# AnnSeidel/genometools

Hardware: AMD Instinct MI355X
Metric: Gbp/s ESA build (suf+lcp+bwt), 3 Gbp DNA, 1/2/4/8 MI355X; bit-exact vs CPU (higher is better)
Workload: dtype u64; 1 GPU; human-like DNA (2% N, 24 seqs, repeats) n=3000000000 seed=43 -suf -lcp -bwt (BASELINE.json configs[2]); parallelism=1 device, pair_suffixes=341032298, tied_suffixes=390540711, refine_rounds=9, maxbranchdepth=8256

## Files before the change

genometools_amd/csrc/esa_engine.hip:

```cpp
#include <stdarg.h>
#include <stdlib.h>
#include <chrono>
#include <type_traits>
#include <utility>
#include <vector>
#include "../../include/gtamd_esa.h"
#include "esa_prims.h"
#include "esa_devutil.h"
#include "esa_own.h"

static thread_local char g_err[1024] = "";
void gtamd_set_error(const char *fmt, ...) {
  va_list ap;
  va_start(ap, fmt);
  vsnprintf(g_err, sizeof g_err, fmt, ap);
  va_end(ap);
}
extern "C" const char *gtamd_esa_last_error(void) { return g_err; }

extern "C" int gtamd_device_count(void) {
  GTAMD_ABI_BEGIN
  int n = 0;
  if (hipGetDeviceCount(&n) != hipSuccess) return 0;
  return n;
// ... 2412 lines not shown
  bool msd_pack = true;
  u32 msd_pack_cap = MD_CAP;
  u32 msd_bin_limit = MD_BIN_LIMIT_DEFAULT;
  bool fused_pass0 = true;
  bool force_wide = false;
  bool no_pairs = false;
  bool no_small_groups = false;
  int apply_early = 2;
  u64 apply_wgs = 0;
  bool apply_wgs_given = false;
  int rank_window_bits = RW_BITS;
  bool rank_all_windows = false;
  bool win_filter_global = false;
  int pair_chunk = 0;
  u32 round_stride = 1536;
  bool debug = false;
};

static Switches read_switches() {
  Switches sw;
  auto flag = [](const char *name, char c) {
    const char *e = getenv(name);
    return e != nullptr && e[0] == c;
  };
  if (const char *e = getenv("GTAMD_MSD")) sw.msd = e[0] == '1';
  sw.msd_part_off = flag("GTAMD_MSD", '0');
  if (const char *e = getenv("GTAMD_MSD_CBITS")) {
    const int v = atoi(e);
    if (v >= 0 && v <= 8) sw.msd_cbits = v;
  }
// ... 23 lines not shown
    sw.apply_wgs_given = true;
  }
  if (const char *e = getenv("GTAMD_RANK_WINDOW_BITS")) {
    const int v = atoi(e);
    if (v >= 2 && v <= RW_BITS) sw.rank_window_bits = v;
  }
  sw.rank_all_windows = flag("GTAMD_RANK_ALL_WINDOWS", '1');
  sw.win_filter_global = flag("GTAMD_WIN_FILTER_LDS", '0');
  if (const char *e = getenv("GTAMD_PAIR_CHUNK")) {
    const int v = atoi(e);
    if (v >= 4 && v <= 1024) sw.pair_chunk = v;
  }
  if (const char *e = getenv("GTAMD_ROUND_STRIDE")) {
    const int v = atoi(e);
    if (v >= RT_STRIDE_MIN && v <= RT_TILE) sw.round_stride = (u32) v;
  }
  sw.debug = getenv("GTAMD_DEBUG") != nullptr;
  return sw;
}

struct gtamd_esa_ctx {
  int device = 0;
  u32 sigma = 0;
  int bits = 0;
  u64 max_n = 0, n = 0, N = 0;
  int readmode = 0;
  Stream st, st2;
  Event ev_sorted, ev_emitted, ev_applied;
  DevBuf tb_own, sp_own;
  Text text = {};
// ... 789 lines not shown
template <int BITS, bool WIDE>
struct Build {
  using K = Key<BITS>;
  using P = typename std::conditional<WIDE, u64, u32>::type;
  static constexpr u64 RANKREC = 1 + sizeof(P) / 4;
  static constexpr u64 ISA_CHUNK = 1ull << 27;

  gtamd_esa_ctx *const c;
  const Switches &sw;
  u32 want;
  const bool dist;
  const u64 N, n;
  const u32 R;
  const hipStream_t st;
  const bool debug;

  u32 prefixlength = 0;
  bool long_prefix = false, want_suf = false, want_lcp = false, want_bwt = false;
  bool msd = false;
  bool msd_part = false;
  bool fused_pass0 = false;

  int fail = 0;

  u64 NL, index_offset = 0;
  Tiles tl;
  u64 Tn;
  u64 prev_key = 0;
  int has_prev = 0;

// ... 141 lines not shown
    u32 *lhead = nullptr;
    u64 list_cap = 0;
  } rk;

  struct RankTable {
    u32 *rank32, *heads, *ppos, *phead, *qhead, *qpos;
    const u32 *spos;
    bool heads_array;
    int wmax, pb, wb, split;
    int fb;
    GroupHeadValues headgen;
  } rt;

  Build(gtamd_esa_ctx *ctx, const Switches &switches, u32 want_, bool dist_)
      : c(ctx), sw(switches), want(want_), dist(dist_), N(ctx->N), n(ctx->n), R(ctx->numparts),
        st(ctx->st), debug(switches.debug), NL(ctx->N), Tn(ctx->N) {
    tl.T = N;
    tl.self = c->part;
  }

  int run() {
    TRY(plan());
    if (!dist) TRY(first_sort_whole());
    else if (msd_part) TRY(first_sort_filtered());
    else TRY(first_sort_exchanged());
    TRY(finish_first_sort());
    TRY(count_ties());
    if (anyties > 0) {
      TRY(count_tied_words());
      bool settled = false;
      TRY(settle_few_ties(&settled));
// ... 33 lines not shown
    TRY(fork_second_stream());
    if (NL > 0) {
      k_finalize<BITS, P><<<stride_grid(div_up(NL, FIN_TILE)), FIN_THREADS, 0, c->st2>>>(
          skey, sa, NL, prefixlength, d_suf, d_lcp, d_bwt, nullptr,
          c->d_stats, prev_key, has_prev, index_offset);
      HIP_TRY(hipGetLastError());
    }
    HIP_TRY(hipEventRecord(c->ev_emitted, c->st2));
    return 0;
  }

  int tie_words(const u64 *bits) {
    if (NL > 0) {
      k_tie_words<<<(u32) nwb, 256, 0, st>>>(bits, nwords, wd.cntw, wd.headw);
      HIP_TRY(hipGetLastError());
      TRY(scan_u32(SCAN_SUM, wd.cntw, wd.offw, nwb, false, wd.scanws, st));
      TRY(scan_u32(SCAN_MAX, wd.headw, wd.carry, nwords, false, wd.scanws, st));
    }
    k_total<<<1, 1, 0, st>>>(wd.offw, wd.cntw, NL > 0 ? nwb : 0, c->d_stats);
    HIP_TRY(hipGetLastError());
    TRY(fetch_stats(c));
    return 0;
  }

  u64 direct_limit() const { return NL / 512 > 4096 ? NL / 512 : 4096; }
  int direct_ties(const u32 *uidx0, const u32 *ugrp, bool clear_fallback) {
    TRY(launch_emission());
    HIP_TRY(hipStreamWaitEvent(st, c->ev_emitted, 0));
    if (clear_fallback) HIP_TRY(hipMemsetAsync(&c->d_stats->dfallback, 0, 4, st));
    if (m0 > 0) {
      k_direct_ties<BITS, P><<<(u32) div_up(m0, 256), 256, 0, st>>>(
          c->text, uidx0, ugrp, m0, sa, d_suf, d_lcp, d_bwt, want_lcp,
// ... 24 lines not shown
    if (R > 1 && (c->comm_allgather == nullptr || c->comm_alltoallv == nullptr)) {
      gtamd_set_error("a part build needs the collective callbacks "
                      "(gtamd_esa_set_comm)");
      return -1;
    }
    memset(&c->timing, 0, sizeof c->timing);
    memset(&c->stats, 0, sizeof c->stats);
    c->alloc_ms = 0;
    c->llv_pairs = 0;
    if (!dist && !WIDE && !(want & GTAMD_WANT_BCK) && N >= 64 && (BITS == 2 || (prefixlength <= 9 && c->sigma <= 20))) {
      msd = sw.msd >= 0 ? sw.msd == 1 : N >= (1ull << 25);
    }
    if (dist && BITS == 2) msd_part = !sw.msd_part_off;
    fused_pass0 = !dist && !msd && BITS == 2 && sw.fused_pass0;
    if (debug)
      fprintf(stderr, "gtamd: part %u: run: parts=%u positions=%d first_sort=%s pass0=%s\n", c->part, R,
              WIDE ? 64 : 32, msd || msd_part ? "msd" : "lsd",
              dist || msd || BITS != 2 ? "none" : (fused_pass0 ? "fused" : "plain"));
    return 0;
  }

  int first_sort_whole() {
    TRY(ensure_workspace(c, N, want, false));
    HIP_TRY(hipMemsetAsync(c->d_stats, 0, sizeof(Stats), st));
    HIP_TRY(hipEventRecord(c->ev[EV_START], st));
    if (msd) {
      TRY(msd_sort_emit<BITS == 5 ? 1 : 0>(c, sw, want, prefixlength, N, N, nullptr, &msd_sa, &msd_fkey, &msd_fval,
                                           &msd_local));
      HIP_TRY(hipEventRecord(c->ev_emitted, st));
    } else if (fused_pass0) {
      const u32 ntiles = (u32) div_up(N, KP_TILE);
      k_dc_hist_dna<<<ntiles, KP_THREADS, 0, st>>>(c->text, N, c->rws.as<u32>());
      HIP_TRY(hipGetLastError());
// ... 51 lines not shown
    if (NL >= SINGLE_LIMIT) {
      set_slice_error(NL);
      return -1;
    }
    const u64 cap = NL > Tn ? NL : Tn;
    TRY(ensure_workspace(c, cap, want, true));
    if (WIDE) TRY(ensure_buf(c, c->posw, (NL + 8) * 8, "the positions of the part's suffixes"));
    msd_sa = c->v0.as<u32>();
    msd_fkey = c->k1.as<u64>();
    msd_fval = c->v1.as<u32>();
    if (NL == 0) {
      HIP_TRY(hipMemsetAsync(c->tiebits.p, 0, 16, st));
      HIP_TRY(hipEventRecord(c->ev[EV_KEYS], st));
      return 0;
    }
    TRY(scan_u32(SCAN_SUM, tkeep, tkeep, ntT, false, tscan, st));
    u64 *ck = c->isa_tmp.as<u64>();
    HIP_TRY(hipMemsetAsync(acc + 3, 0, 8, st));
    if (WIDE)
      k_part_filter<u64><<<ntT, MS_THREADS, 0, st>>>(c->text, N, lo, hi, binbelow, tkeep, ck,
                                                    c->posw.as<u64>(), acc + 3);
    else
      k_part_filter<u32><<<ntT, MS_THREADS, 0, st>>>(c->text, N, lo, hi, binbelow, tkeep, ck,
                                                    c->v1.as<u32>(), acc + 3);
    HIP_TRY(hipGetLastError());
    MsdPartSrc src;
    src.ck = ck;
    src.cp32 = WIDE ? nullptr : c->v1.as<u32>();
    src.index_offset = index_offset;
    src.prev_key = acc + 3;
    src.has_prev = has_prev;
// ... 111 lines not shown
              (unsigned long long) index_offset, WIDE ? " (64-bit positions)" : "");
    if (dist && !msd_part) TRY(comm_allgather(c, fail, nullptr, nullptr, 0));
    if (!msd) HIP_TRY(hipEventRecord(c->ev[EV_KEYS], st));

    static_assert((64 - Key<2>::LOW_BITS) % 8 == 0, "whole passes over the DNA prefix");
    int shifts[16], widths[16];
    const int np = passes_for(pass0_done ? K::LOW_BITS : K::DSHIFT, 64, shifts, widths);
    u64 *ka = pass0_done ? c->k1.as<u64>() : c->k0.as<u64>(),
        *kb = pass0_done ? c->k0.as<u64>() : c->k1.as<u64>();
    u32 *va = pass0_done ? c->v1.as<u32>() : c->v0.as<u32>(),
        *vb = pass0_done ? c->v0.as<u32>() : c->v1.as<u32>();
    if (!msd) {
      hipEvent_t evs[2 * 16];
      for (int i = 0; i < 2 * 16; i++) evs[i] = c->ev_scatter[i];
      TRY(radix_sort_pairs<u64, u32>(ka, va, kb, vb, NL, shifts, widths, np,
                                c->rws.as<u32>(), st, evs, &nev));
    }
    skey = (np & 1) ? kb : ka;
    u32 *sa32 = (np & 1) ? vb : va;
    fkey = (np & 1) ? ka : kb;
    fval = (np & 1) ? va : vb;
    if (msd) {
      skey = nullptr;
      sa32 = msd_sa;
      fkey = msd_fkey;
      fval = msd_fval;
    }
    HIP_TRY(hipEventRecord(c->ev[EV_SORTED], st));

    if (want & GTAMD_WANT_BCK) TRY(build_bcktab<BITS>(c, skey, sa32, NL, prefixlength, st));

// ... 82 lines not shown
    return 0;
  }

  int pair_path() {
    TRY(ensure_buf(c, c->tiebits2, (nwords + 2) * 8, "the tie bitmap"));
    tiebits2 = c->tiebits2.as<u64>();
    const bool no_pairs = sw.no_pairs;
    const bool no_small = no_pairs || sw.no_small_groups;
    u64 nsrec = 0;
    if (NL > 0) {
      if (no_pairs) {
        HIP_TRY(hipMemcpyAsync(tiebits2, tiebits, nwords * 8, hipMemcpyDeviceToDevice, st));
      } else {
        k_pair_words<<<(u32) nwb, 256, 0, st>>>(tiebits, nwords, wd.pcnt, wd.scnt, wd.rcnt, tiebits2);
        HIP_TRY(hipGetLastError());
        TRY(scan_u32(SCAN_SUM, wd.pcnt, wd.poff, nwb, false, wd.scanws, st));
        TRY(scan_u32(SCAN_SUM, wd.scnt, wd.soff, nwb, false, wd.scanws, st));
        TRY(scan_u32(SCAN_SUM, wd.rcnt, wd.roff, nwb, false, wd.scanws, st));
        k_total2<<<1, 1, 0, st>>>(wd.poff, wd.pcnt, nwb, c->d_stats);
        k_total3<<<1, 1, 0, st>>>(wd.soff, wd.scnt, nwb, c->d_stats);
        k_total<<<1, 1, 0, st>>>(wd.roff, wd.rcnt, nwb, c->d_stats);
        HIP_TRY(hipGetLastError());
        TRY(fetch_stats(c));
        npairs = c->h_stats->count2;
        nsmall = c->h_stats->count3;
        nsrec = c->h_stats->count;
      }
    }
    if (no_small || nsrec > NL / 8 || npairs + nsrec >= SINGLE_LIMIT) { nsmall = 0; nsrec = 0; }
    nrec = npairs + nsrec;
    apply_early = sw.apply_early;
    {
      Bump sz = {nullptr, 0};
// ... 10 lines not shown
    nbl = bits_for(NL ? NL - 1 : 0);
    pn = passes_for(0, nb, ps, pw);
    pair_swp = npairs > 0 ? pl.swp : nullptr;
    if (nrec == 0) return 0;
    if (npairs > 0) {
      k_pair_emit<P><<<(u32) div_up(nwords, 256), 256, 0, st>>>(tiebits, nwords, wd.poff, sa, pl.pk_a,
                                                               pl.pv_a, pl.pidx);
      HIP_TRY(hipGetLastError());
    }
    if (nsmall > 0) {
      k_small_emit<P><<<(u32) div_up(nwords, 256), 256, 0, st>>>(
          tiebits, nwords, wd.soff, wd.roff, sa, npairs, pl.sidx, pl.ssize, pl.srec, pl.pk_a, pl.pv_a);
      HIP_TRY(hipGetLastError());
    }
    TRY(radix_sort_pairs<P, u64>(pl.pk_a, pl.pv_a, pl.pk_b, pl.pv_b, nrec, ps, pw, pn, pl.prws, st,
                                 nullptr, nullptr));
    const P *pk_sorted = (pn & 1) ? pl.pk_b : pl.pk_a;
    const u64 *pv_sorted = (pn & 1) ? pl.pv_b : pl.pv_a;
    TRY(launch_emission());
    int pair_chunk = (int) (nrec >> 20 < 16 ? 16 : (nrec >> 20 > 128 ? 128 : nrec >> 20));
    if (sw.pair_chunk > 0) pair_chunk = sw.pair_chunk;
    pair_chunk = (pair_chunk + PR_LINE - 1) / PR_LINE * PR_LINE;
    if (debug)
      fprintf(stderr, "gtamd: part %u: pair resolve: records=%llu chunk=%d grid=%u\n", c->part,
              (unsigned long long) nrec, pair_chunk,
              stride_grid(div_up(div_up(nrec, (u64) pair_chunk), 256)));
    k_pair_resolve<BITS, P><<<stride_grid(div_up(div_up(nrec, (u64) pair_chunk), 256)), 256, 0, st>>>(
        c->text, pk_sorted, pv_sorted, nrec, npairs, sa, pl.pres, c->d_stats, pair_chunk);
    HIP_TRY(hipGetLastError());
    if (npairs > 0) {
      k_pair_swapbits<<<(u32) nwb, 256, 0, st>>>(tiebits, nwords, wd.poff, pl.pres, pl.swp);
// ... 160 lines not shown
  int rank_windows(const u32 *in_pos, const u32 *in_head, u32 *a_pos, u32 *a_head, u32 *b_pos,
                   u32 *b_head, u64 count, int bits, int pb, int split, u64 span, const u32 *list,
                   int fb, u32 nsel, u64 M) {
    const u32 *wpos = in_pos, *whead = in_head;
    if (pb > 0) {
      const int s0 = bits - pb, w0 = pb > 8 ? pb - 8 : pb;
      if (in_head != nullptr)
        TRY(radix_partition_u32(in_pos, in_head, a_pos, a_head, count, s0, w0, wd.pws, st));
      else
        TRY(radix_pass_group_heads(in_pos, rt.headgen, a_pos, a_head, count, s0, w0, wd.pws, st));
      wpos = a_pos; whead = a_head;
    }
    if (pb > 8) {
      const int s1 = bits - 8, w1 = 8;
      TRY(radix_sort_pairs<u32, u32>(a_pos, a_head, b_pos, b_head, count, &s1, &w1, 1, wd.pws, st,
                                     nullptr, nullptr));
      wpos = b_pos; whead = b_head;
    }
    const int wb = bits - pb;
    const u32 nbuckets = (u32) div_up(count, 1ull << wb);
    const u32 grid = split == 2 ? ((nbuckets + 7u) / 8u) * 16u : nbuckets;
    k_rank_window<<<grid, RW_THREADS, 0, st>>>(wpos, whead, span, wb, split, nbuckets, rt.rank32,
                                               list, fb, nsel, M);
    HIP_TRY(hipGetLastError());
    return 0;
  }

  int build_rank(bool first) {
    u64 nsel = 0;
    if (rk.windows) {
      k_win_select<<<1, 1024, 0, st>>>(rk.w_need, rk.w_built, rk.nww, rk.w_sel, rk.w_list, rk.w_pref, c->d_stats);
// ... 331 lines not shown
      if (c->h_stats->count2 != 0) TRY(build_rank(false));
    }
    const u32 rt_stride = sw.round_stride;
    const u32 g = (u32) div_up(m, 256);
    const u32 ntiles = (u32) div_up(m, rt_stride);
    const u32 nfb = (u32) div_up(m, RT_TILE);
    u32 *tilecnt = ar.koff, *tileoff = ar.koff + nfb + 16;
    HIP_TRY(hipMemsetAsync(ar.flagbits, 0, (u64) nfb * (RT_TILE / 8), st));
    k_tile_starts<<<ntiles / 256 + 1, 256, 0, st>>>(ar.ugrp, m, ntiles, rt_stride, ar.tstart);
    HIP_TRY(hipGetLastError());
    k_round_tile<P><<<ntiles, RT_THREADS, 0, st>>>(
        ar.uidx, ar.upos, ar.ugrp, ar.k2, m, ar.cvo, ar.hv, ar.tstart, ar.flagbits, dist ? nullptr : rank, h, n);
    HIP_TRY(hipGetLastError());
    k_flag_count<<<nfb / 256 + 1, 256, 0, st>>>(ar.flagbits, m, nfb, tilecnt);
    HIP_TRY(hipGetLastError());
    TRY(scan_u32(SCAN_SUM, tilecnt, tileoff, nfb, false, ar.scanws2, st));
    k_total<<<1, 1, 0, st>>>(tileoff, tilecnt, nfb, c->d_stats);
    HIP_TRY(hipGetLastError());
    TRY(fetch_stats(c));
    const u64 nf = c->h_stats->count;
    if (debug)
      fprintf(stderr, "gtamd: part %u round %u: %llu entries in groups across tile borders "
              "(%u tiles, stride %u)\n", c->part, rounds, (unsigned long long) nf, ntiles, rt_stride);
    if (nf > 0) {
      k_flag_gather<P><<<nfb, RT_THREADS, 0, st>>>(ar.flagbits, tileoff, ar.ugrp, ar.k2, ar.upos, m, ar.fk2,
                                                     ar.fk2s_a, ar.fgrp, ar.fpos, ar.fj, ar.perm_a);
      HIP_TRY(hipGetLastError());
      TRY(radix_sort_pairs<P, u32>(ar.fk2s_a, ar.perm_a, ar.fk2s_b, ar.perm_b, nf, ps, pw, pn, ar.rws2, st,
                                   nullptr, nullptr));
      u32 *perm1 = (pn & 1) ? ar.perm_b : ar.perm_a, *permx = (pn & 1) ? ar.perm_a : ar.perm_b;
      const u32 gf = (u32) div_up(nf, 256);
      k_gather_u32<<<gf, 256, 0, st>>>(ar.fgrp, perm1, nf, ar.gk_a);
      HIP_TRY(hipGetLastError());
      TRY(radix_sort_pairs<u32, u32>(ar.gk_a, perm1, ar.gk_b, permx, nf, s.gs, s.gw, s.gn, ar.rws2, st,
                                     nullptr, nullptr));
      const u32 *perm2 = (s.gn & 1) ? permx : perm1;
      k_flag_heads<P><<<gf, 256, 0, st>>>(perm2, ar.fgrp, ar.fk2, ar.fpos, ar.uidx, ar.fj, nf, ar.fhv, ar.cvs);
      HIP_TRY(hipGetLastError());
      TRY(scan_u32(SCAN_MAX, ar.fhv, ar.fhv, nf, true, ar.scanws2, st));
      k_flag_scatter<P><<<gf, 256, 0, st>>>(ar.cvs, ar.fhv, ar.fj, nf, ar.cvo, ar.hv);
      HIP_TRY(hipGetLastError());
    }
    u32 *bcnt = ar.koff, *boffs = ar.koff + g + 16;
    k_round_apply<P><<<g, 256, 0, st>>>(ar.cvo, ar.hv, ar.uidx, ar.ugrp, m, index_offset, sa,
                                        dist ? nullptr : rank, ar.keep, bcnt);
    HIP_TRY(hipGetLastError());
    TRY(scan_u32(SCAN_SUM, bcnt, boffs, g, false, ar.scanws2, st));
    k_round_compact<P><<<g, 256, 0, st>>>(ar.keep, boffs, bcnt, ar.uidx, ar.cvo, ar.hv, m, ar.uidx2,
                                          ar.upos2, ar.ugrp2, c->d_stats);
    HIP_TRY(hipGetLastError());
    TRY(fetch_stats(c));
    s.m = c->h_stats->count;
    s.h *= 2;
    if (dist) {
      s.ru.cval = ar.cvo; s.ru.gnew = ar.hv; s.ru.ugrp = ar.ugrp; s.ru.index_offset = index_offset;
      s.ru.tl = tl; s.ru.isa = isa; s.ru.soff = ar.xoff; s.ru.srank = ar.xrank;
      s.m_upd = m;
      TRY(dest_count(c, s.ru, s.m_upd, ar.xdest_u, ar.xbc_u, ar.xbo_u, ar.scanws2, 1));
      s.rq.upos = ar.upos2; s.rq.h = s.h;
      TRY(dest_count(c, s.rq, s.m, ar.xdest_q, ar.xbc_q, ar.xbo_q, ar.scanws2, 0));
    }
    std::swap(ar.uidx, ar.uidx2);
// ... 12 lines not shown
      else lcpfull = c->isa_tmp.as<u32>();
    }
    if (!apply_early) TRY(launch_apply(st));
    const u32 g0 = (u32) div_up(m0, 256);
    u32 *bcnt0 = ar.koff, *boff0 = ar.koff + g0 + 16;
    if (m0 > 0) {
      TRY(fork_second_stream());
      k_fix_basic<BITS, P><<<g0, 256, 0, c->st2>>>(c->text, ar.uidx0, m0, sa, d_suf, d_bwt,
                                                   c->d_stats, index_offset);
      HIP_TRY(hipGetLastError());
      HIP_TRY(hipEventRecord(c->ev_emitted, c->st2));
    }
    if (want_lcp && m0 > 0) {
      k_tied_counts<<<g0, 256, 0, st>>>(ar.uidx0, m0, tiebits2, bcnt0);
      HIP_TRY(hipGetLastError());
      TRY(scan_u32(SCAN_SUM, bcnt0, boff0, g0, false, ar.scanws2, st));
      k_total<<<1, 1, 0, st>>>(boff0, bcnt0, g0, c->d_stats);
      HIP_TRY(hipGetLastError());
      TRY(fetch_stats(c));
      const u64 m1 = c->h_stats->count;
      k_lcp_pairs<P><<<g0, 256, 0, st>>>(boff0, tiebits2, ar.uidx0, sa, m0, ar.lk_a, ar.lv_a);
      HIP_TRY(hipGetLastError());
      TRY(radix_sort_pairs<P, u32>(ar.lk_a, ar.lv_a, ar.lk_b, ar.lv_b, m1, ps, pw, pn, ar.rws2, st,
                                   nullptr, nullptr));
      const P *pk = (pn & 1) ? ar.lk_b : ar.lk_a;
      const u32 *pv = (pn & 1) ? ar.lv_b : ar.lv_a;
      k_lcp_chunks<BITS, P><<<stride_grid(div_up(div_up(m1, LCP_CHUNK), 256)), 256, 0, st>>>(
          c->text, pk, pv, m1, sa, d_lcp, lcpfull, c->d_stats);
      HIP_TRY(hipGetLastError());
    }
    if (apply_early) HIP_TRY(hipStreamWaitEvent(st, c->ev_applied, 0));
    if (!want_lcp) return 0;
    TRY(fetch_stats(c));
    const u64 pairs = c->h_stats->numlarge;
    if (pairs * 16 > c->llv.bytes) HIP_TRY(c->llv.alloc((pairs + pairs / 4 + 1024) * 16));
    if (pairs > 0) {
      const u32 gl = (u32) div_up(NL, LLV_TILE);
      u32 *lc = wd.cntw, *lo = wd.offw;
      k_large_counts<<<gl, 256, 0, st>>>(d_lcp, NL, lc);
      HIP_TRY(hipGetLastError());
      TRY(scan_u32(SCAN_SUM, lc, lo, gl, false, wd.scanws, st));
      k_llv_emit<<<gl, 256, 0, st>>>(d_lcp, NL, lcpfull, lo, index_offset, c->llv);
      HIP_TRY(hipGetLastError());
    }
    c->llv_pairs = pairs;
    return 0;
  }

  int report() {
    TRY(launch_emission());
    HIP_TRY(hipStreamWaitEvent(st, c->ev_emitted, 0));
    HIP_TRY(hipEventRecord(c->ev[EV_DONE], st));
    TRY(fetch_stats(c));

    c->stats.totallength = n;
    c->stats.numberofallsortedsuffixes = N;
// ... 223 lines not shown
```

genometools_amd/csrc/esa_prims.h:

```cpp
#pragma once
#include "esa_common.h"

enum { SCAN_SUM = 0, SCAN_MAX = 1 };

u64 scan_workspace_words(u64 n);
int scan_u32(int op, const u32 *in, u32 *out, u64 n, bool inclusive, u32 *ws,
             hipStream_t st);

int offsets_u64(const u32 *cnt, u64 count, u64 *tsum, u64 *off, u64 *total_dev, hipStream_t st);
int offsets_u64_counted(const u32 *cnt, u64 count, u64 *tsum, u64 *off, u64 *total_dev, hipStream_t st);

u64 radix_workspace_words(u64 n);
template <typename K, typename V>
int radix_sort_pairs(K *keys_a, V *vals_a, K *keys_b, V *vals_b, u64 n,
                     const int *shifts, const int *widths, int npasses,
                     u32 *ws, hipStream_t st, hipEvent_t *ev_pairs,
                     int *n_ev);

int radix_scan_tile_hist(u32 *ws, u64 n, hipStream_t st);
u64 radix_rows_workspace_words(u64 nrows);
int radix_scan_tile_rows(u32 *hist, u32 nrows, u32 *scanws, hipStream_t st);

struct GroupHeadValues {
  const u64 *tiebits;
  const u32 *carry;
  u64 nwords;
  u32 offset;
  const u64 *swp;
};
int radix_pass_group_heads(const u32 *keys_a, GroupHeadValues gen, u32 *keys_b,
                           u32 *vals_b, u64 n, int shift, int width, u32 *ws,
                           hipStream_t st);
// ... 4 lines not shown
```

genometools_amd/csrc/esa_prims.hip:

```cpp
#include "esa_prims.h"
#include "esa_devutil.h"

namespace {

constexpr int SC_ITEMS = 16;
constexpr int SC_TILE = SC_THREADS * SC_ITEMS;

template <int OP>
__global__ __launch_bounds__(SC_THREADS) void k_scan_reduce(
    const u32 *__restrict__ in, u64 n, u32 *__restrict__ blocksum) {
  __shared__ u32 lds4[4];
  const u64 base = (u64) blockIdx.x * SC_TILE + (u64) threadIdx.x * SC_ITEMS;
  u32 acc = 0;
#pragma unroll
  for (int i = 0; i < SC_ITEMS; i++) {
    u64 idx = base + i;
    if (idx < n) acc = sc_op<OP>(acc, in[idx]);
  }
  u32 tot;
  (void) block_scan_excl<OP>(acc, &tot, lds4);
  if (threadIdx.x == 0) blocksum[blockIdx.x] = tot;
}

template <int OP, bool INCLUSIVE>
// ... 10 lines not shown
    v[i] = idx < n ? in[idx] : 0;
    acc = sc_op<OP>(acc, v[i]);
  }
  u32 tot;
  u32 pre = block_scan_excl<OP>(acc, &tot, lds4);
  if (blockprefix != nullptr) pre = sc_op<OP>(pre, blockprefix[blockIdx.x]);
#pragma unroll
  for (int i = 0; i < SC_ITEMS; i++) {
    u64 idx = base + i;
    u32 incl = sc_op<OP>(pre, v[i]);
    if (idx < n) out[idx] = INCLUSIVE ? incl : pre;
    pre = incl;
  }
}

}

u64 scan_workspace_words(u64 n) {
  u64 words = 0;
  while (n > SC_TILE) {
    n = div_up(n, SC_TILE);
    words += n + 16;
  }
  return words + 16;
}

template <int OP>
static int scan_rec(const u32 *in, u32 *out, u64 n, bool inclusive, u32 *ws,
                    hipStream_t st) {
  if (n == 0) return 0;
  const u64 nblocks = div_up(n, SC_TILE);
  if (nblocks == 1) {
    if (inclusive)
      k_scan_tile<OP, true><<<1, SC_THREADS, 0, st>>>(in, out, n, nullptr);
    else
      k_scan_tile<OP, false><<<1, SC_THREADS, 0, st>>>(in, out, n, nullptr);
    HIP_TRY(hipGetLastError());
    return 0;
  }
  u32 *sums = ws;
  k_scan_reduce<OP><<<(u32) nblocks, SC_THREADS, 0, st>>>(in, n, sums);
  HIP_TRY(hipGetLastError());
  TRY(scan_rec<OP>(sums, sums, nblocks, false, ws + nblocks + 16, st));
  if (inclusive)
    k_scan_tile<OP, true><<<(u32) nblocks, SC_THREADS, 0, st>>>(in, out, n, sums);
  else
    k_scan_tile<OP, false><<<(u32) nblocks, SC_THREADS, 0, st>>>(in, out, n, sums);
  HIP_TRY(hipGetLastError());
  return 0;
}

int scan_u32(int op, const u32 *in, u32 *out, u64 n, bool inclusive, u32 *ws,
             hipStream_t st) {
  return op == SCAN_SUM ? scan_rec<SCAN_SUM>(in, out, n, inclusive, ws, st)
                        : scan_rec<SCAN_MAX>(in, out, n, inclusive, ws, st);
}

namespace {

__global__ __launch_bounds__(SC_THREADS) void k_scan64(u64 *a, u64 count, u64 *total) {
  __shared__ u64 s[SC_THREADS];
  block_scan_excl_array_u64(a, count, total, s);
}

__global__ __launch_bounds__(SC_THREADS) void k_offsets(const u32 *cnt, const u64 *tsum, u64 count, u64 *off) {
  __shared__ u64 s[SC_THREADS];
  const u64 i = (u64) blockIdx.x * SC_THREADS + threadIdx.x;
  const u64 v = i < count ? cnt[i] : 0;
  const u64 incl = block_scan_incl_u64(v, s) + tsum[blockIdx.x];
  if (i < count) {
// ... 298 lines not shown
  __shared__ u16 s_cnt[RS_WAVES * RADIX];
  __shared__ u32 s_obase[RADIX];
  static_assert(sizeof(K) * RS_TILE + sizeof(V) * RS_TILE + sizeof(u16) * RS_WAVES * RADIX
                + sizeof(u32) * RADIX <= 53 * 1024 || sizeof(K) + sizeof(V) > 12,
                "three workgroups per CU");

  const int tid = threadIdx.x;
  const u32 tile = xcd_tile(blockIdx.x, ntiles);
  if (tile >= ntiles) return;
  const u64 tile_base = (u64) tile * RS_TILE;
  const u32 valid = tile + 1u == ntiles ? last_valid : (u32) RS_TILE;
  for (int i = tid; i < RS_WAVES * RADIX / 2; i += RS_THREADS)
    reinterpret_cast<u32 *>(s_cnt)[i] = 0;
  u32 gbase = 0;
  if (tid < RADIX) gbase = hist_scanned[(u64) tile * RADIX + tid];
  if (valid == (u32) RS_TILE)
    rs_scatter_tile<true, K, V>(keys_in + tile_base, vals_in + tile_base, keys_out, vals_out,
                                valid, shift, mask, gbase, s_key, s_val, s_cnt, s_obase);
  else
    rs_scatter_tile<false, K, V>(keys_in + tile_base, vals_in + tile_base, keys_out, vals_out,
                                 valid, shift, mask, gbase, s_key, s_val, s_cnt, s_obase);
}

template <bool FULL, typename K, typename V, typename VG>
__device__ __forceinline__ void rs_partition_tile(
    const K *__restrict__ keys_in, const V *__restrict__ vals_in,
    K *__restrict__ keys_out, V *__restrict__ vals_out, const u32 valid, int shift,
    u32 mask, u32 gbase, K *s_key, V *s_val, u32 *s_cnt ,
    u32 *s_obase, u32 *s_scan, const VG vg, u64 first) {
  const int tid = threadIdx.x, lane = tid & 63, w = tid >> 6;
// ... 90 lines not shown
}

static u64 cs_workspace_words(u64 ntiles) {
  return (ntiles / CS_ROWS + 2) * RADIX;
}

u64 radix_workspace_words(u64 n) {
  u64 ntiles = div_up(n, RS_TILE);
  u64 hist = ntiles * RADIX;
  return hist + cs_workspace_words(ntiles) + 64;
}

template <typename K, typename V>
int radix_sort_pairs(K *keys_a, V *vals_a, K *keys_b, V *vals_b, u64 n,
                     const int *shifts, const int *widths, int npasses,
                     u32 *ws, hipStream_t st, hipEvent_t *ev_pairs, int *n_ev) {
  if (n == 0) return 0;
  if (n >= (1ull << 32)) {
    gtamd_set_error("radix_sort_pairs: %llu pairs exceed the 32-bit index "
                    "range of one sort", (unsigned long long) n);
    return -1;
  }
  const u32 ntiles = (u32) div_up(n, RS_TILE);
  const u32 last_valid = (u32) (n - (u64) (ntiles - 1) * RS_TILE);
  u32 *hist = ws;
  u32 *scanws = ws + (u64) ntiles * RADIX;
  K *kin = keys_a, *kout = keys_b;
  V *vin = vals_a, *vout = vals_b;
  for (int p = 0; p < npasses; p++) {
    const u32 mask = (1u << widths[p]) - 1u;
    k_rs_hist<K><<<ntiles, RS_THREADS, 0, st>>>(kin, n, shifts[p], mask, hist, ntiles);
    HIP_TRY(hipGetLastError());
    TRY(radix_scan_tile_rows(hist, ntiles, scanws, st));
    if (ev_pairs != nullptr) HIP_TRY(hipEventRecord(ev_pairs[2 * *n_ev], st));
    k_rs_scatter<K, V><<<((ntiles + 7u) >> 3) * 8u, RS_THREADS, 0, st>>>(
        kin, vin, kout, vout, last_valid, shifts[p], mask, hist, ntiles);
    HIP_TRY(hipGetLastError());
    if (ev_pairs != nullptr) {
      HIP_TRY(hipEventRecord(ev_pairs[2 * *n_ev + 1], st));
      (*n_ev)++;
    }
    K *tk = kin; kin = kout; kout = tk;
    V *tv = vin; vin = vout; vout = tv;
  }
  return 0;
}

int radix_pass_group_heads(const u32 *keys_a, GroupHeadValues gen, u32 *keys_b,
                           u32 *vals_b, u64 n, int shift, int width, u32 *ws,
                           hipStream_t st) {
  if (n == 0) return 0;
  if (n >= (1ull << 32)) {
// ... 42 lines not shown

u64 radix_rows_workspace_words(u64 nrows) { return cs_workspace_words(nrows) + 64; }

int radix_scan_tile_rows(u32 *hist, u32 ntiles, u32 *scanws, hipStream_t st) {
  if (ntiles == 0) return 0;
  const u32 nchunks = (ntiles + CS_ROWS - 1) / CS_ROWS;
  k_cs_chunksum<<<nchunks, RADIX, 0, st>>>(hist, ntiles, scanws);
  HIP_TRY(hipGetLastError());
  k_cs_chunkbase<<<1, RADIX * CB_PARTS, 0, st>>>(scanws, nchunks);
  HIP_TRY(hipGetLastError());
  k_cs_rows<<<nchunks, RADIX, 0, st>>>(hist, ntiles, scanws);
  HIP_TRY(hipGetLastError());
  return 0;
}

template int radix_sort_pairs<u64, u32>(u64 *, u32 *, u64 *, u32 *, u64, const int *,
                                        const int *, int, u32 *, hipStream_t, hipEvent_t *,
                                        int *);
template int radix_sort_pairs<u32, u32>(u32 *, u32 *, u32 *, u32 *, u64, const int *,
                                        const int *, int, u32 *, hipStream_t, hipEvent_t *,
                                        int *);
template int radix_sort_pairs<u32, u64>(u32 *, u64 *, u32 *, u64 *, u64, const int *,
                                        const int *, int, u32 *, hipStream_t, hipEvent_t *,
                                        int *);
template int radix_sort_pairs<u64, u64>(u64 *, u64 *, u64 *, u64 *, u64, const int *,
                                        const int *, int, u32 *, hipStream_t, hipEvent_t *,
                                        int *);
```

Before: 26.73 Gbp/s.

## Add single-launch small-input paths for scans and radix sort passes

Adds a single-kernel scan for inputs up to a threshold, where each block recomputes its own prefix carry by reducing all preceding elements instead of running the reduce, recursive-scan and tile kernels. Adds a fused radix pass for small sorts in which each tile counts digits over the whole input itself, replacing the separate histogram, three-kernel row scan and scatter launches. The aim is fewer kernel launches and dependent steps in the many small refinement-round sorts and scans. The cost is redundant work that grows with the number of tiles, so the thresholds are exposed as environment switches. The flag-scatter scan also now writes to a separate buffer, because the small scan path needs non-aliased input and output.

```diff
diff --git a/genometools_amd/csrc/esa_engine.hip b/genometools_amd/csrc/esa_engine.hip
--- a/genometools_amd/csrc/esa_engine.hip
+++ b/genometools_amd/csrc/esa_engine.hip
@@ -2450,6 +2450,8 @@
   bool win_filter_global = false;
   int pair_chunk = 0;
   u32 round_stride = 1536;
+  u64 small_sort = PRIM_SMALL_SORT_DEFAULT;
+  u64 small_scan = PRIM_SMALL_SCAN_DEFAULT;
   bool debug = false;
 };
 
@@ -2503,6 +2505,14 @@
   if (const char *e = getenv("GTAMD_ROUND_STRIDE")) {
     const int v = atoi(e);
     if (v >= RT_STRIDE_MIN && v <= RT_TILE) sw.round_stride = (u32) v;
+  }
+  if (const char *e = getenv("GTAMD_SMALL_SORT")) {
+    const long long v = atoll(e);
+    if (v >= 0 && v <= (long long) PRIM_SMALL_SORT_CAP) sw.small_sort = (u64) v;
+  }
+  if (const char *e = getenv("GTAMD_SMALL_SCAN")) {
+    const long long v = atoll(e);
+    if (v >= 0 && v <= (long long) PRIM_SMALL_SCAN_CAP) sw.small_scan = (u64) v;
   }
   sw.debug = getenv("GTAMD_DEBUG") != nullptr;
   return sw;
@@ -3322,6 +3332,7 @@
   const u32 R;
   const hipStream_t st;
   const bool debug;
+  const PrimTuning tune;
 
   u32 prefixlength = 0;
   bool long_prefix = false, want_suf = false, want_lcp = false, want_bwt = false;
@@ -3493,7 +3504,8 @@
 
   Build(gtamd_esa_ctx *ctx, const Switches &switches, u32 want_, bool dist_)
       : c(ctx), sw(switches), want(want_), dist(dist_), N(ctx->N), n(ctx->n), R(ctx->numparts),
-        st(ctx->st), debug(switches.debug), NL(ctx->N), Tn(ctx->N) {
+        st(ctx->st), debug(switches.debug), tune{switches.small_sort, switches.small_scan, nullptr},
+        NL(ctx->N), Tn(ctx->N) {
     tl.T = N;
     tl.self = c->part;
   }
@@ -3557,8 +3569,8 @@
     if (NL > 0) {
       k_tie_words<<<(u32) nwb, 256, 0, st>>>(bits, nwords, wd.cntw, wd.headw);
       HIP_TRY(hipGetLastError());
-      TRY(scan_u32(SCAN_SUM, wd.cntw, wd.offw, nwb, false, wd.scanws, st));
-      TRY(scan_u32(SCAN_MAX, wd.headw, wd.carry, nwords, false, wd.scanws, st));
+      TRY(scan_u32(SCAN_SUM, wd.cntw, wd.offw, nwb, false, wd.scanws, st, &tune));
+      TRY(scan_u32(SCAN_MAX, wd.headw, wd.carry, nwords, false, wd.scanws, st, &tune));
     }
     k_total<<<1, 1, 0, st>>>(wd.offw, wd.cntw, NL > 0 ? nwb : 0, c->d_stats);
     HIP_TRY(hipGetLastError());
@@ -3613,9 +3625,11 @@
     if (dist && BITS == 2) msd_part = !sw.msd_part_off;
     fused_pass0 = !dist && !msd && BITS == 2 && sw.fused_pass0;
     if (debug)
-      fprintf(stderr, "gtamd: part %u: run: parts=%u positions=%d first_sort=%s pass0=%s\n", c->part, R,
+      fprintf(stderr, "gtamd: part %u: run: parts=%u positions=%d first_sort=%s pass0=%s "
+              "small_sort=%llu small_scan=%llu\n", c->part, R,
               WIDE ? 64 : 32, msd || msd_part ? "msd" : "lsd",
-              dist || msd || BITS != 2 ? "none" : (fused_pass0 ? "fused" : "plain"));
+              dist || msd || BITS != 2 ? "none" : (fused_pass0 ? "fused" : "plain"),
+              (unsigned long long) tune.small_sort, (unsigned long long) tune.small_scan);
     return 0;
   }
 
@@ -3697,7 +3711,7 @@
       HIP_TRY(hipEventRecord(c->ev[EV_KEYS], st));
       return 0;
     }
-    TRY(scan_u32(SCAN_SUM, tkeep, tkeep, ntT, false, tscan, st));
+    TRY(scan_u32(SCAN_SUM, tkeep, tkeep, ntT, false, tscan, st, &tune));
     u64 *ck = c->isa_tmp.as<u64>();
     HIP_TRY(hipMemsetAsync(acc + 3, 0, 8, st));
     if (WIDE)
@@ -3839,7 +3853,7 @@
       hipEvent_t evs[2 * 16];
       for (int i = 0; i < 2 * 16; i++) evs[i] = c->ev_scatter[i];
       TRY(radix_sort_pairs<u64, u32>(ka, va, kb, vb, NL, shifts, widths, np,
-                                c->rws.as<u32>(), st, evs, &nev));
+                                c->rws.as<u32>(), st, evs, &nev, &tune));
     }
     skey = (np & 1) ? kb : ka;
     u32 *sa32 = (np & 1) ? vb : va;
@@ -3952,9 +3966,9 @@
       } else {
         k_pair_words<<<(u32) nwb, 256, 0, st>>>(tiebits, nwords, wd.pcnt, wd.scnt, wd.rcnt, tiebits2);
         HIP_TRY(hipGetLastError());
-        TRY(scan_u32(SCAN_SUM, wd.pcnt, wd.poff, nwb, false, wd.scanws, st));
-        TRY(scan_u32(SCAN_SUM, wd.scnt, wd.soff, nwb, false, wd.scanws, st));
-        TRY(scan_u32(SCAN_SUM, wd.rcnt, wd.roff, nwb, false, wd.scanws, st));
+        TRY(scan_u32(SCAN_SUM, wd.pcnt, wd.poff, nwb, false, wd.scanws, st, &tune));
+        TRY(scan_u32(SCAN_SUM, wd.scnt, wd.soff, nwb, false, wd.scanws, st, &tune));
+        TRY(scan_u32(SCAN_SUM, wd.rcnt, wd.roff, nwb, false, wd.scanws, st, &tune));
         k_total2<<<1, 1, 0, st>>>(wd.poff, wd.pcnt, nwb, c->d_stats);
         k_total3<<<1, 1, 0, st>>>(wd.soff, wd.scnt, nwb, c->d_stats);
         k_total<<<1, 1, 0, st>>>(wd.roff, wd.rcnt, nwb, c->d_stats);
@@ -3995,7 +4009,7 @@
       HIP_TRY(hipGetLastError());
     }
     TRY(radix_sort_pairs<P, u64>(pl.pk_a, pl.pv_a, pl.pk_b, pl.pv_b, nrec, ps, pw, pn, pl.prws, st,
-                                 nullptr, nullptr));
+                                 nullptr, nullptr, &tune));
     const P *pk_sorted = (pn & 1) ? pl.pk_b : pl.pk_a;
     const u64 *pv_sorted = (pn & 1) ? pl.pv_b : pl.pv_a;
     TRY(launch_emission());
@@ -4186,7 +4200,7 @@
     if (pb > 8) {
       const int s1 = bits - 8, w1 = 8;
       TRY(radix_sort_pairs<u32, u32>(a_pos, a_head, b_pos, b_head, count, &s1, &w1, 1, wd.pws, st,
-                                     nullptr, nullptr));
+                                     nullptr, nullptr, &tune));
       wpos = b_pos; whead = b_head;
     }
     const int wb = bits - pb;
@@ -4548,7 +4562,7 @@
     HIP_TRY(hipGetLastError());
     k_flag_count<<<nfb / 256 + 1, 256, 0, st>>>(ar.flagbits, m, nfb, tilecnt);
     HIP_TRY(hipGetLastError());
-    TRY(scan_u32(SCAN_SUM, tilecnt, tileoff, nfb, false, ar.scanws2, st));
+    TRY(scan_u32(SCAN_SUM, tilecnt, tileoff, nfb, false, ar.scanws2, st, &tune));
     k_total<<<1, 1, 0, st>>>(tileoff, tilecnt, nfb, c->d_stats);
     HIP_TRY(hipGetLastError());
     TRY(fetch_stats(c));
@@ -4561,25 +4575,25 @@
                                                      ar.fk2s_a, ar.fgrp, ar.fpos, ar.fj, ar.perm_a);
       HIP_TRY(hipGetLastError());
       TRY(radix_sort_pairs<P, u32>(ar.fk2s_a, ar.perm_a, ar.fk2s_b, ar.perm_b, nf, ps, pw, pn, ar.rws2, st,
-                                   nullptr, nullptr));
+                                   nullptr, nullptr, &tune));
       u32 *perm1 = (pn & 1) ? ar.perm_b : ar.perm_a, *permx = (pn & 1) ? ar.perm_a : ar.perm_b;
       const u32 gf = (u32) div_up(nf, 256);
       k_gather_u32<<<gf, 256, 0, st>>>(ar.fgrp, perm1, nf, ar.gk_a);
       HIP_TRY(hipGetLastError());
       TRY(radix_sort_pairs<u32, u32>(ar.gk_a, perm1, ar.gk_b, permx, nf, s.gs, s.gw, s.gn, ar.rws2, st,
-                                     nullptr, nullptr));
+                                     nullptr, nullptr, &tune));
       const u32 *perm2 = (s.gn & 1) ? permx : perm1;
       k_flag_heads<P><<<gf, 256, 0, st>>>(perm2, ar.fgrp, ar.fk2, ar.fpos, ar.uidx, ar.fj, nf, ar.fhv, ar.cvs);
       HIP_TRY(hipGetLastError());
-      TRY(scan_u32(SCAN_MAX, ar.fhv, ar.fhv, nf, true, ar.scanws2, st));
-      k_flag_scatter<P><<<gf, 256, 0, st>>>(ar.cvs, ar.fhv, ar.fj, nf, ar.cvo, ar.hv);
+      TRY(scan_u32(SCAN_MAX, ar.fhv, ar.gk_a, nf, true, ar.scanws2, st, &tune));
+      k_flag_scatter<P><<<gf, 256, 0, st>>>(ar.cvs, ar.gk_a, ar.fj, nf, ar.cvo, ar.hv);
       HIP_TRY(hipGetLastError());
     }
     u32 *bcnt = ar.koff, *boffs = ar.koff + g + 16;
     k_round_apply<P><<<g, 256, 0, st>>>(ar.cvo, ar.hv, ar.uidx, ar.ugrp, m, index_offset, sa,
                                         dist ? nullptr : rank, ar.keep, bcnt);
     HIP_TRY(hipGetLastError());
-    TRY(scan_u32(SCAN_SUM, bcnt, boffs, g, false, ar.scanws2, st));
+    TRY(scan_u32(SCAN_SUM, bcnt, boffs, g, false, ar.scanws2, st, &tune));
     k_round_compact<P><<<g, 256, 0, st>>>(ar.keep, boffs, bcnt, ar.uidx, ar.cvo, ar.hv, m, ar.uidx2,
                                           ar.upos2, ar.ugrp2, c->d_stats);
     HIP_TRY(hipGetLastError());
@@ -4622,7 +4636,7 @@
     if (want_lcp && m0 > 0) {
       k_tied_counts<<<g0, 256, 0, st>>>(ar.uidx0, m0, tiebits2, bcnt0);
       HIP_TRY(hipGetLastError());
-      TRY(scan_u32(SCAN_SUM, bcnt0, boff0, g0, false, ar.scanws2, st));
+      TRY(scan_u32(SCAN_SUM, bcnt0, boff0, g0, false, ar.scanws2, st, &tune));
       k_total<<<1, 1, 0, st>>>(boff0, bcnt0, g0, c->d_stats);
       HIP_TRY(hipGetLastError());
       TRY(fetch_stats(c));
@@ -4630,7 +4644,7 @@
       k_lcp_pairs<P><<<g0, 256, 0, st>>>(boff0, tiebits2, ar.uidx0, sa, m0, ar.lk_a, ar.lv_a);
       HIP_TRY(hipGetLastError());
       TRY(radix_sort_pairs<P, u32>(ar.lk_a, ar.lv_a, ar.lk_b, ar.lv_b, m1, ps, pw, pn, ar.rws2, st,
-                                   nullptr, nullptr));
+                                   nullptr, nullptr, &tune));
       const P *pk = (pn & 1) ? ar.lk_b : ar.lk_a;
       const u32 *pv = (pn & 1) ? ar.lv_b : ar.lv_a;
       k_lcp_chunks<BITS, P><<<stride_grid(div_up(div_up(m1, LCP_CHUNK), 256)), 256, 0, st>>>(
@@ -4647,7 +4661,7 @@
       u32 *lc = wd.cntw, *lo = wd.offw;
       k_large_counts<<<gl, 256, 0, st>>>(d_lcp, NL, lc);
       HIP_TRY(hipGetLastError());
-      TRY(scan_u32(SCAN_SUM, lc, lo, gl, false, wd.scanws, st));
+      TRY(scan_u32(SCAN_SUM, lc, lo, gl, false, wd.scanws, st, &tune));
       k_llv_emit<<<gl, 256, 0, st>>>(d_lcp, NL, lcpfull, lo, index_offset, c->llv);
       HIP_TRY(hipGetLastError());
     }
diff --git a/genometools_amd/csrc/esa_prims.h b/genometools_amd/csrc/esa_prims.h
--- a/genometools_amd/csrc/esa_prims.h
+++ b/genometools_amd/csrc/esa_prims.h
@@ -3,9 +3,21 @@
 
 enum { SCAN_SUM = 0, SCAN_MAX = 1 };
 
+struct PrimTuning {
+  u64 small_sort;
+  u64 small_scan;
+  u32 *launches;
+};
+constexpr u64 PRIM_SMALL_SORT_DEFAULT = 1ull << 15;
+constexpr u64 PRIM_SMALL_SCAN_DEFAULT = 1ull << 17;
+constexpr u64 PRIM_SMALL_SORT_CAP = 1ull << 20;
+constexpr u64 PRIM_SMALL_SCAN_CAP = 1ull << 20;
+
 u64 scan_workspace_words(u64 n);
 int scan_u32(int op, const u32 *in, u32 *out, u64 n, bool inclusive, u32 *ws,
              hipStream_t st);
+int scan_u32(int op, const u32 *in, u32 *out, u64 n, bool inclusive, u32 *ws,
+             hipStream_t st, const PrimTuning *tune);
 
 int offsets_u64(const u32 *cnt, u64 count, u64 *tsum, u64 *off, u64 *total_dev, hipStream_t st);
 int offsets_u64_counted(const u32 *cnt, u64 count, u64 *tsum, u64 *off, u64 *total_dev, hipStream_t st);
@@ -16,6 +28,11 @@
                      const int *shifts, const int *widths, int npasses,
                      u32 *ws, hipStream_t st, hipEvent_t *ev_pairs,
                      int *n_ev);
+template <typename K, typename V>
+int radix_sort_pairs(K *keys_a, V *vals_a, K *keys_b, V *vals_b, u64 n,
+                     const int *shifts, const int *widths, int npasses,
+                     u32 *ws, hipStream_t st, hipEvent_t *ev_pairs,
+                     int *n_ev, const PrimTuning *tune);
 
 int radix_scan_tile_hist(u32 *ws, u64 n, hipStream_t st);
 u64 radix_rows_workspace_words(u64 nrows);
diff --git a/genometools_amd/csrc/esa_prims.hip b/genometools_amd/csrc/esa_prims.hip
--- a/genometools_amd/csrc/esa_prims.hip
+++ b/genometools_amd/csrc/esa_prims.hip
@@ -48,6 +48,54 @@
   }
 }
 
+template <int OP, bool INCLUSIVE>
+__global__ __launch_bounds__(SC_THREADS) void k_scan_small(
+    const u32 *__restrict__ in, u32 *__restrict__ out, u32 n) {
+  __shared__ u32 lds4[4];
+  const u32 tid = threadIdx.x;
+  const u32 front = blockIdx.x * (u32) SC_TILE;
+  u32 head = (u32) ((16u - (u32) (reinterpret_cast<uintptr_t>(in) & 15u)) & 15u) / 4u;
+  head = head < front ? head : front;
+  const u32 nq = (front - head) / 4u, tail = front - head - 4u * nq;
+  u32 acc = 0;
+  if (tid < head) acc = in[tid];
+  if (tid < tail) acc = sc_op<OP>(acc, in[head + 4u * nq + tid]);
+  const uint4 *q = reinterpret_cast<const uint4 *>(in + head);
+  u32 i = tid;
+  for (; i + 7u * SC_THREADS < nq; i += 8u * SC_THREADS) {
+    uint4 v[8];
+#pragma unroll
+    for (int k = 0; k < 8; k++) v[k] = q[i + (u32) k * SC_THREADS];
+#pragma unroll
+    for (int k = 0; k < 8; k++)
+      acc = sc_op<OP>(acc, sc_op<OP>(sc_op<OP>(v[k].x, v[k].y), sc_op<OP>(v[k].z, v[k].w)));
+  }
+  for (; i < nq; i += SC_THREADS) {
+    const uint4 v = q[i];
+    acc = sc_op<OP>(acc, sc_op<OP>(sc_op<OP>(v.x, v.y), sc_op<OP>(v.z, v.w)));
+  }
+  u32 carry;
+  (void) block_scan_excl<OP>(acc, &carry, lds4);
+  const u32 base = front + tid * SC_ITEMS;
+  u32 v[SC_ITEMS];
+  acc = 0;
+#pragma unroll
+  for (int k = 0; k < SC_ITEMS; k++) {
+    const u32 idx = base + k;
+    v[k] = idx < n ? in[idx] : 0;
+    acc = sc_op<OP>(acc, v[k]);
+  }
+  u32 tot;
+  u32 pre = sc_op<OP>(block_scan_excl<OP>(acc, &tot, lds4), carry);
+#pragma unroll
+  for (int k = 0; k < SC_ITEMS; k++) {
+    const u32 idx = base + k;
+    const u32 incl = sc_op<OP>(pre, v[k]);
+    if (idx < n) out[idx] = INCLUSIVE ? incl : pre;
+    pre = incl;
+  }
+}
+
 }
 
 u64 scan_workspace_words(u64 n) {
@@ -59,9 +107,20 @@
   return words + 16;
 }
 
+static PrimTuning prim_limits(const PrimTuning *tune) {
+  PrimTuning t = {PRIM_SMALL_SORT_DEFAULT, PRIM_SMALL_SCAN_DEFAULT, nullptr};
+  if (tune != nullptr) t = *tune;
+  if (t.small_sort > PRIM_SMALL_SORT_CAP) t.small_sort = PRIM_SMALL_SORT_CAP;
+  if (t.small_scan > PRIM_SMALL_SCAN_CAP) t.small_scan = PRIM_SMALL_SCAN_CAP;
+  return t;
+}
+static inline void count_launch(const PrimTuning &t) {
+  if (t.launches != nullptr) ++*t.launches;
+}
+
 template <int OP>
 static int scan_rec(const u32 *in, u32 *out, u64 n, bool inclusive, u32 *ws,
-                    hipStream_t st) {
+                    hipStream_t st, const PrimTuning &t) {
   if (n == 0) return 0;
   const u64 nblocks = div_up(n, SC_TILE);
   if (nblocks == 1) {
@@ -70,24 +129,42 @@
     else
       k_scan_tile<OP, false><<<1, SC_THREADS, 0, st>>>(in, out, n, nullptr);
     HIP_TRY(hipGetLastError());
+    count_launch(t);
+    return 0;
+  }
+  if (n <= t.small_scan && (in + n <= out || out + n <= in)) {
+    if (inclusive)
+      k_scan_small<OP, true><<<(u32) nblocks, SC_THREADS, 0, st>>>(in, out, (u32) n);
+    else
+      k_scan_small<OP, false><<<(u32) nblocks, SC_THREADS, 0, st>>>(in, out, (u32) n);
+    HIP_TRY(hipGetLastError());
+    count_launch(t);
     return 0;
   }
   u32 *sums = ws;
   k_scan_reduce<OP><<<(u32) nblocks, SC_THREADS, 0, st>>>(in, n, sums);
   HIP_TRY(hipGetLastError());
-  TRY(scan_rec<OP>(sums, sums, nblocks, false, ws + nblocks + 16, st));
+  count_launch(t);
+  TRY(scan_rec<OP>(sums, sums, nblocks, false, ws + nblocks + 16, st, t));
   if (inclusive)
     k_scan_tile<OP, true><<<(u32) nblocks, SC_THREADS, 0, st>>>(in, out, n, sums);
   else
     k_scan_tile<OP, false><<<(u32) nblocks, SC_THREADS, 0, st>>>(in, out, n, sums);
   HIP_TRY(hipGetLastError());
+  count_launch(t);
   return 0;
+}
+
+int scan_u32(int op, const u32 *in, u32 *out, u64 n, bool inclusive, u32 *ws,
+             hipStream_t st, const PrimTuning *tune) {
+  const PrimTuning t = prim_limits(tune);
+  return op == SCAN_SUM ? scan_rec<SCAN_SUM>(in, out, n, inclusive, ws, st, t)
+                        : scan_rec<SCAN_MAX>(in, out, n, inclusive, ws, st, t);
 }
 
 int scan_u32(int op, const u32 *in, u32 *out, u64 n, bool inclusive, u32 *ws,
              hipStream_t st) {
-  return op == SCAN_SUM ? scan_rec<SCAN_SUM>(in, out, n, inclusive, ws, st)
-                        : scan_rec<SCAN_MAX>(in, out, n, inclusive, ws, st);
+  return scan_u32(op, in, out, n, inclusive, ws, st, nullptr);
 }
 
 namespace {
@@ -416,6 +493,82 @@
     reinterpret_cast<u32 *>(s_cnt)[i] = 0;
   u32 gbase = 0;
   if (tid < RADIX) gbase = hist_scanned[(u64) tile * RADIX + tid];
+  if (valid == (u32) RS_TILE)
+    rs_scatter_tile<true, K, V>(keys_in + tile_base, vals_in + tile_base, keys_out, vals_out,
+                                valid, shift, mask, gbase, s_key, s_val, s_cnt, s_obase);
+  else
+    rs_scatter_tile<false, K, V>(keys_in + tile_base, vals_in + tile_base, keys_out, vals_out,
+                                 valid, shift, mask, gbase, s_key, s_val, s_cnt, s_obase);
+}
+
+
+template <typename K>
+__device__ __forceinline__ void rs_count_keys(const K *__restrict__ keys, u32 lo, u32 hi,
+                                              int shift, u32 mask, u32 *hrow) {
+  constexpr u32 PER = 16 / sizeof(K);
+  const u32 tid = threadIdx.x;
+  const K *kp = keys + lo;
+  u32 head = (PER - (u32) ((reinterpret_cast<uintptr_t>(kp) / sizeof(K)) & (PER - 1u))) & (PER - 1u);
+  head = head < hi - lo ? head : hi - lo;
+  const u32 nq = (hi - lo - head) / PER, tail = hi - lo - head - PER * nq;
+  if (tid < head) atomicAdd(&hrow[(u32) (kp[tid] >> shift) & mask], 1u);
+  if (tid < tail) atomicAdd(&hrow[(u32) (kp[head + PER * nq + tid] >> shift) & mask], 1u);
+  const uint4 *q = reinterpret_cast<const uint4 *>(kp + head);
+  auto count4 = [&](const uint4 v) {
+    if (sizeof(K) == 8) {
+      atomicAdd(&hrow[(u32) ((((u64) v.y << 32) | v.x) >> shift) & mask], 1u);
+      atomicAdd(&hrow[(u32) ((((u64) v.w << 32) | v.z) >> shift) & mask], 1u);
+    } else {
+      atomicAdd(&hrow[(v.x >> shift) & mask], 1u);
+      atomicAdd(&hrow[(v.y >> shift) & mask], 1u);
+      atomicAdd(&hrow[(v.z >> shift) & mask], 1u);
+      atomicAdd(&hrow[(v.w >> shift) & mask], 1u);
+    }
+  };
+  u32 i = tid;
+  for (; i + 7u * RS_THREADS < nq; i += 8u * RS_THREADS) {
+    uint4 v[8];
+#pragma unroll
+    for (int k = 0; k < 8; k++) v[k] = q[i + (u32) k * RS_THREADS];
+#pragma unroll
+    for (int k = 0; k < 8; k++) count4(v[k]);
+  }
+  for (; i < nq; i += RS_THREADS) count4(q[i]);
+}
+
+template <typename K, typename V>
+__global__ __launch_bounds__(RS_THREADS) void k_rs_small_pass(
+    const K *__restrict__ keys_in, const V *__restrict__ vals_in,
+    K *__restrict__ keys_out, V *__restrict__ vals_out, u32 n, u32 last_valid, int shift,
+    u32 mask, u32 ntiles) {
+  __shared__ K s_key[RS_TILE];
+  __shared__ V s_val[RS_TILE];
+  __shared__ u16 s_cnt[RS_WAVES * RADIX];
+  __shared__ u32 s_obase[RADIX];
+  static_assert(sizeof(K) * RS_TILE >= 2 * sizeof(u32) * RS_WAVES * RADIX, "two histograms in s_key");
+  const int tid = threadIdx.x, w = tid >> 6;
+  const u32 tile = blockIdx.x;
+  const u32 tile_base = tile * (u32) RS_TILE;
+  const u32 valid = tile + 1u == ntiles ? last_valid : (u32) RS_TILE;
+  u32 *h_before = reinterpret_cast<u32 *>(s_key), *h_after = h_before + RS_WAVES * RADIX;
+  for (int i = tid; i < 2 * RS_WAVES * RADIX; i += RS_THREADS) h_before[i] = 0;
+  for (int i = tid; i < RS_WAVES * RADIX / 2; i += RS_THREADS)
+    reinterpret_cast<u32 *>(s_cnt)[i] = 0;
+  __syncthreads();
+  rs_count_keys<K>(keys_in, 0u, tile_base, shift, mask, h_before + w * RADIX);
+  rs_count_keys<K>(keys_in, tile_base, n, shift, mask, h_after + w * RADIX);
+  __syncthreads();
+  u32 before = 0, total = 0;
+  if (tid < RADIX) {
+#pragma unroll
+    for (int i = 0; i < RS_WAVES; i++) {
+      before += h_before[i * RADIX + tid];
+      total += h_after[i * RADIX + tid];
+    }
+    total += before;
+  }
+  u32 all;
+  const u32 gbase = block_scan_excl<SCAN_SUM, RS_THREADS>(total, &all, s_obase) + before;
   if (valid == (u32) RS_TILE)
     rs_scatter_tile<true, K, V>(keys_in + tile_base, vals_in + tile_base, keys_out, vals_out,
                                 valid, shift, mask, gbase, s_key, s_val, s_cnt, s_obase);
@@ -536,28 +689,39 @@
 template <typename K, typename V>
 int radix_sort_pairs(K *keys_a, V *vals_a, K *keys_b, V *vals_b, u64 n,
                      const int *shifts, const int *widths, int npasses,
-                     u32 *ws, hipStream_t st, hipEvent_t *ev_pairs, int *n_ev) {
+                     u32 *ws, hipStream_t st, hipEvent_t *ev_pairs, int *n_ev,
+                     const PrimTuning *tune) {
   if (n == 0) return 0;
   if (n >= (1ull << 32)) {
     gtamd_set_error("radix_sort_pairs: %llu pairs exceed the 32-bit index "
                     "range of one sort", (unsigned long long) n);
     return -1;
   }
+  const PrimTuning t = prim_limits(tune);
+  const bool small = n <= t.small_sort;
   const u32 ntiles = (u32) div_up(n, RS_TILE);
   const u32 last_valid = (u32) (n - (u64) (ntiles - 1) * RS_TILE);
   u32 *hist = ws;
-  u32 *scanws = ws + (u64) ntiles * RADIX;
+  u32 *scanws = small ? nullptr : ws + (u64) ntiles * RADIX;
   K *kin = keys_a, *kout = keys_b;
   V *vin = vals_a, *vout = vals_b;
   for (int p = 0; p < npasses; p++) {
     const u32 mask = (1u << widths[p]) - 1u;
-    k_rs_hist<K><<<ntiles, RS_THREADS, 0, st>>>(kin, n, shifts[p], mask, hist, ntiles);
+    if (!small) {
+      k_rs_hist<K><<<ntiles, RS_THREADS, 0, st>>>(kin, n, shifts[p], mask, hist, ntiles);
+      HIP_TRY(hipGetLastError());
+      TRY(radix_scan_tile_rows(hist, ntiles, scanws, st));
+      if (t.launches != nullptr) *t.launches += 4;
+    }
+    if (ev_pairs != nullptr) HIP_TRY(hipEventRecord(ev_pairs[2 * *n_ev], st));
+    if (small)
+      k_rs_small_pass<K, V><<<ntiles, RS_THREADS, 0, st>>>(kin, vin, kout, vout, (u32) n, last_valid,
+                                                         shifts[p], mask, ntiles);
+    else
+      k_rs_scatter<K, V><<<((ntiles + 7u) >> 3) * 8u, RS_THREADS, 0, st>>>(
+          kin, vin, kout, vout, last_valid, shifts[p], mask, hist, ntiles);
     HIP_TRY(hipGetLastError());
-    TRY(radix_scan_tile_rows(hist, ntiles, scanws, st));
-    if (ev_pairs != nullptr) HIP_TRY(hipEventRecord(ev_pairs[2 * *n_ev], st));
-    k_rs_scatter<K, V><<<((ntiles + 7u) >> 3) * 8u, RS_THREADS, 0, st>>>(
-        kin, vin, kout, vout, last_valid, shifts[p], mask, hist, ntiles);
-    HIP_TRY(hipGetLastError());
+    count_launch(t);
     if (ev_pairs != nullptr) {
       HIP_TRY(hipEventRecord(ev_pairs[2 * *n_ev + 1], st));
       (*n_ev)++;
@@ -630,15 +794,22 @@
   return 0;
 }
 
-template int radix_sort_pairs<u64, u32>(u64 *, u32 *, u64 *, u32 *, u64, const int *,
-                                        const int *, int, u32 *, hipStream_t, hipEvent_t *,
-                                        int *);
-template int radix_sort_pairs<u32, u32>(u32 *, u32 *, u32 *, u32 *, u64, const int *,
-                                        const int *, int, u32 *, hipStream_t, hipEvent_t *,
-                                        int *);
-template int radix_sort_pairs<u32, u64>(u32 *, u64 *, u32 *, u64 *, u64, const int *,
-                                        const int *, int, u32 *, hipStream_t, hipEvent_t *,
-                                        int *);
-template int radix_sort_pairs<u64, u64>(u64 *, u64 *, u64 *, u64 *, u64, const int *,
-                                        const int *, int, u32 *, hipStream_t, hipEvent_t *,
-                                        int *);
+template <typename K, typename V>
+int radix_sort_pairs(K *keys_a, V *vals_a, K *keys_b, V *vals_b, u64 n,
+                     const int *shifts, const int *widths, int npasses,
+                     u32 *ws, hipStream_t st, hipEvent_t *ev_pairs, int *n_ev) {
+  return radix_sort_pairs<K, V>(keys_a, vals_a, keys_b, vals_b, n, shifts, widths, npasses, ws, st,
+                                ev_pairs, n_ev, nullptr);
+}
+
+#define RS_INSTANCE(K, V)                                                                  \
+  template int radix_sort_pairs<K, V>(K *, V *, K *, V *, u64, const int *, const int *,   \
+                                      int, u32 *, hipStream_t, hipEvent_t *, int *);       \
+  template int radix_sort_pairs<K, V>(K *, V *, K *, V *, u64, const int *, const int *,   \
+                                      int, u32 *, hipStream_t, hipEvent_t *, int *,        \
+                                      const PrimTuning *);
+RS_INSTANCE(u64, u32)
+RS_INSTANCE(u32, u32)
+RS_INSTANCE(u32, u64)
+RS_INSTANCE(u64, u64)
+#undef RS_INSTANCE
```

Result: slower. 26.40 Gbp/s (-1.2%).
